# JeffOwOSun/ntm-tracker

Measured on AMD Instinct MI355X. Metric: frames/sec (whole node) VGG16+NTM(128x20) seq_len=20, higher is better.
Workload: dtype f32

## Files before the change

### ntm-tracker_amd/csrc/ntm_phases.h

```cpp
#pragma once
#include "ntm_fwd_args.h"

struct NtmCtl {
    int O, oK, oB, oG, oS, oY, oE, oA, P, PP, ldz, ldh, write_first;
};

__device__ __forceinline__ NtmCtl ntm_ctl(int Md, int R, int Wh, int hid, int SS, int O, int write_first) {
    const int H = R + Wh, K = R * Md + hid;
    NtmCtl d;
    d.O = O;
    d.oK = 0; d.oB = H * Md; d.oG = d.oB + H; d.oS = d.oG + H; d.oY = d.oS + H * SS; d.oE = d.oY + H;
    d.oA = d.oE + Wh * Md; d.P = d.oA + Wh * Md;
    d.PP = (d.P + d.O + 3) & ~3; d.ldz = (K + 1 + 3) & ~3; d.ldh = (hid + 1 + 3) & ~3;
    d.write_first = write_first;
    return d;
}

struct NtmFwdSt {
    int T, N, Md, MP, R, Wh, H, hid, SS, RM;
    int nslB, kperB;
    int nslR, nperR;
    float *sPart, *sM, *sW, *sWg, *sZ, *sU, *sKs, *sPw;
    float* sCn;
    const float* sH;
};

__device__ __forceinline__ NtmFwdSt ntm_fwd_state(float* smem, const NtmLds& L, int T, int N, int Md, int R, int Wh, int hid,
                                                  int SS, int PP, int h_at) {
    NtmFwdSt c;
    c.T = T; c.N = N; c.Md = Md; c.MP = Md | 1; c.R = R; c.Wh = Wh; c.H = R + Wh; c.hid = hid; c.SS = SS; c.RM = R * Md;
    c.nslB = min(max(1, T / (PP >> 2)), hid);
    c.kperB = (hid + c.nslB - 1) / c.nslB;
    c.nslR = min(max(1, T / c.RM), N);
    c.nperR = (N + c.nslR - 1) / c.nslR;
    c.sPart = smem + L.part; c.sM = smem + L.M; c.sW = smem + L.W; c.sWg = smem + L.Wg; c.sZ = smem + L.Z; c.sU = smem + L.U;
    c.sKs = smem + L.Ks; c.sCn = smem + L.Cn; c.sPw = smem + L.Pw;
    c.sH = c.sZ + h_at;
    return c;
}

template <bool SMOOTH>
__device__ __forceinline__ void ntm_fwd_mem_norms(const NtmFwdSt& c, int tid) {
    const int N = c.N, Md = c.Md, MP = c.MP, lane = tid & 63, wave = tid >> 6, nwaves = c.T >> 6;
    const int w0 = (c.hid + 63) >> 6;
    if constexpr (SMOOTH) {
        if (wave >= w0) {
            for (int n = (wave - w0) * 64 + lane; n < N; n += (nwaves - w0) * 64) {
                float s = 0.f;
                for (int m = 0; m < Md; ++m) { const float v = c.sM[n * MP + m]; s += v * v; }
                c.sCn[n] = sqrtf(s);
            }
        }
    } else
    if (wave >= w0) {
        for (int m = wave - w0; m < Md; m += nwaves - w0) {
            float s = 0.f;
            for (int n = lane; n < N; n += 64) { const float v = c.sM[n * MP + m]; s += v * v; }
            s = wave_sum(s);
            if (lane == 0) c.sCn[m] = 1.0f / sqrtf(fmaxf(s, 1e-12f));
        }
    }
}

template <int NB>
__device__ __forceinline__ void ntm_fwd_unpack_partials(const NtmFwdSt& c, const NtmCtl& d, const f32x4* Wa4, int tid) {
    const int ncg = d.PP >> 2;
    if (tid < c.nslB * ncg) {
        const int cg = tid % ncg, ks = tid / ncg;
        const int k0 = ks * c.kperB, k1 = min(c.hid, k0 + c.kperB);
        reinterpret_cast<f32x4*>(c.sPart)[ks * ncg + cg] = ntk_stream_matvec<NB>(Wa4 + cg, ncg, c.sH, k0, k1, c.hid);
    }
}

__device__ __forceinline__ void ntm_fwd_controls(const NtmFwdSt& c, const NtmCtl& d, const NtmFwdArgs& a, int tid, size_t bt) {
    const int hid = c.hid, nslB = c.nslB, PP = d.PP;
    if (tid < PP) {
        float v = a.Wa[(size_t)hid * PP + tid];
        for (int ks = 0; ks < nslB; ++ks) v += c.sPart[ks * PP + tid];
        float r = v;
        if (tid < d.oB) r = ntm_tanh(v);
        else if (tid < d.oG) r = ntm_softplus(v);
        else if (tid < d.oS) r = ntm_sigmoid(v);
        else if (tid < d.oY) r = v;
        else if (tid < d.oE) r = ntm_softplus(v) + 1.0f;
        else if (tid < d.oA) r = ntm_sigmoid(v);
        else if (tid < d.P) r = ntm_tanh(v);
        c.sU[tid] = r;
        if (a.st_u) a.st_u[bt * PP + tid] = r;
        if (tid >= d.P && tid < d.P + d.O) a.logits[bt * d.O + (tid - d.P)] = v;
    }
}

template <bool SMOOTH, int MAXSS>
__device__ __forceinline__ void ntm_fwd_head_wave(const NtmFwdSt& c, const NtmCtl& d, const NtmFwdArgs& a, int h, int lane, size_t bt) {
    const int N = c.N, Md = c.Md, MP = c.MP, H = c.H, SS = c.SS;
    float kss = 0.f;
    for (int m = 0; m < Md; ++m) { const float kv = c.sU[d.oK + h * Md + m]; kss += kv * kv; }
    const float kn = sqrtf(kss);
    if constexpr (SMOOTH) {
        for (int m = lane; m < Md; m += 64) c.sKs[h * Md + m] = c.sU[d.oK + h * Md + m];
    } else {
        const float kinv = 1.0f / sqrtf(fmaxf(kss, 1e-12f));
        if (lane < Md) c.sKs[h * Md + lane] = c.sU[d.oK + h * Md + lane] * kinv * c.sCn[lane];
        for (int m = lane + 64; m < Md; m += 64) c.sKs[h * Md + m] = c.sU[d.oK + h * Md + m] * kinv * c.sCn[m];
    }
    const float beta = c.sU[d.oB + h], g = c.sU[d.oG + h], gamma = c.sU[d.oY + h];
    float swv[MAXSS];
    {
        float mx = -INFINITY;
#pragma unroll
        for (int j = 0; j < MAXSS; ++j) if (j < SS) mx = fmaxf(mx, c.sU[d.oS + h * SS + j]);
        float sum = 0.f;
#pragma unroll
        for (int j = 0; j < MAXSS; ++j) { swv[j] = (j < SS) ? ntm_exp(c.sU[d.oS + h * SS + j] - mx) : 0.f; sum += swv[j]; }
#pragma unroll
        for (int j = 0; j < MAXSS; ++j) swv[j] = swv[j] / sum;
    }
    __builtin_amdgcn_fence(__ATOMIC_ACQ_REL, "wavefront");
    __builtin_amdgcn_wave_barrier();
    float mxv = -INFINITY;
// ... 169 lines not shown
    if (tid < hid) {
        p.G = reinterpret_cast<const f32x4*>(a.st_gates)[bt * hid + tid];
        p.Ct = a.st_c[bt * hid + tid];
        p.Cp = (t > 0) ? a.st_c[(bt - 1) * hid + tid] : c_init[tid];
    }
}

__device__ __forceinline__ void ntm_bwd_commit(const NtmBwdSt& c, const NtmCtl& d, const NtmBwdWho& w, const NtmBwdRecs& p) {
    const int T = c.T, NMd = c.NMd, Md = c.Md, MP = c.MP, hid = c.hid, PP = d.PP, tid = w.tid;
    const bool hn = w.hn, wf = d.write_first != 0;
#pragma unroll
    for (int q = 0; q < MAXM; ++q) {
        const int idx = tid + q * T;
        if (idx < NMd) {
            const int n = idx / Md, m = idx - n * Md;
            c.sMp[n * MP + m] = p.M[q];
            if (wf) c.sMt[n * MP + m] = p.Mt[q];
        }
    }
    if (hn) { c.sWp[tid] = p.Wp; c.sWt[tid] = p.Wt; c.sWc[tid] = p.Wc; c.sWv[tid] = p.Wv; }
    if (tid < PP) { c.sU[tid] = p.U; c.sDU[tid] = p.Dl; }
    if (tid < hid) { reinterpret_cast<f32x4*>(c.sGt)[tid] = p.G; c.sCt[tid] = p.Ct; c.sCp[tid] = p.Cp; }
}

template <class Args>
__device__ __forceinline__ void ntm_bwd_init_carried(const NtmBwdSt& c, const Args& a, int tid) {
    const int b = c.b, T = c.T, NMd = c.NMd, HN = c.HN, Md = c.Md, MP = c.MP, RM = c.R * c.Md;
    for (int i = tid; i < NMd; i += T)
        c.sdM[(i / Md) * MP + (i % Md)] = a.dM_fin ? a.dM_fin[(size_t)b * NMd + i] : 0.f;
    for (int i = tid; i < HN; i += T) c.sdW[i] = a.dw_fin ? a.dw_fin[(size_t)b * HN + i] : 0.f;
    for (int i = tid; i < RM; i += T) c.sdZ[i] = a.dread_fin ? a.dread_fin[(size_t)b * RM + i] : 0.f;
}

template <int NQS>
__device__ __forceinline__ void ntm_red_write(const NtmBwdSt& c, const NtmBwdWho& w, const float (&v)[NQ], int nq, int base) {
#pragma unroll
    for (int q = 0; q < NQ; ++q) {
        if (q < nq) {
            const float s = wave_sum(w.hn ? v[q] : 0.f);
            if (w.hn && w.lane == 0) c.sRed[(w.hh * NQS + base + q) * c.NW + w.wi] = s;
        }
    }
}

template <int NQS>
__device__ __forceinline__ float ntm_red_read(const NtmBwdSt& c, int h, int q) {
    float s = 0.f;
    for (int w = 0; w < c.NW; ++w) s += c.sRed[(h * NQS + q) * c.NW + w];
    return s;
}

template <int MAXT, bool FIX, bool SMOOTH, class Args, class Barrier, class Stamp>
__device__ __forceinline__ void ntm_bwd_heads_step(const NtmBwdSt& c, const NtmCtl& d, const Args& a, const NtmBwdWho& w, size_t bt,
                                                   Barrier&& barrier, Stamp&& stamp) {
    constexpr int NQS = NQT + (SMOOTH ? 1 : 0);
    const int T = c.T, N = c.N, Md = c.Md, MP = c.MP, R = c.R, Wh = c.Wh, H = c.H, SS = c.SS, NMd = c.NMd, PP = d.PP;
    const int nout = c.nout, nslP = c.nslP, nperP = c.nperP, hg4 = c.hg4, nslH = c.nslH, nperH = c.nperH, nslC = c.nslC, nperC = c.nperC;
    const int tid = w.tid, lane = w.lane, hh = w.hh, nn = w.nn;
    const bool hn = w.hn, wf = d.write_first != 0;
    float* const sPart = c.sPart; float* const sdM = c.sdM; float* const sG = c.sG; float* const sMp = c.sMp; float* const sMt = c.sMt;
    float* const sdW = c.sdW; float* const sWp = c.sWp; float* const sWt = c.sWt; float* const sWc = c.sWc; float* const sWv = c.sWv;
    float* const sWg = c.sWg; float* const sDwv = c.sDwv; float* const sDsim = c.sDsim; float* const sU = c.sU; float* const sDU = c.sDU;
    float* const sdZ = c.sdZ; float* const sKhat = c.sKhat; float* const sKs = c.sKs; float* const sKinv = c.sKinv; float* const sKss = c.sKss;
    float* const sCinv = c.sCinv; float* const sCss = c.sCss; float* const sC2 = c.sC2; float* const sDkhat = c.sDkhat;
    float* const sSw = c.sSw; float* const sDmh = c.sDmh;
    const f32x4* const sWaRes4 = c.sWaRes4;
    float* const sRn = sCinv; float* const sRc = sC2;
    f32x4* const sPart4 = reinterpret_cast<f32x4*>(sPart);

    if constexpr (FIX) {
        const int n = tid / 5, m0 = (tid - n * 5) * 4;
        float wt[5];
#pragma unroll
        for (int i = 0; i < 5; ++i) wt[i] = sWt[i * N + n];
        f32x4 dmr = {0.f, 0.f, 0.f, 0.f};
#pragma unroll
        for (int i = 0; i < 4; ++i) dmr += wt[i] * *reinterpret_cast<const f32x4*>(sdZ + i * Md + m0);
#pragma unroll
        for (int e = 0; e < 4; ++e) {
            const int ai = n * MP + m0 + e;
            const float dMt = sdM[ai];
            const float E = 1.0f - wt[4] * sU[d.oE + m0 + e];
            sG[ai] = dMt;
            sdM[ai] = dMt * E + dmr[e];
        }
    } else
    for (int idx = tid; idx < NMd; idx += T) {
        const int n = idx / Md, m = idx - n * Md, ai = n * MP + m;
        float dMt = sdM[ai];
        float dMr = 0.f;
        for (int i = 0; i < R; ++i) dMr += sWt[i * N + n] * sdZ[i * Md + m];
        if (wf) dMt += dMr;
        float E = 1.f;
        for (int j = 0; j < Wh; ++j) E *= (1.0f - sWt[(R + j) * N + n] * sU[d.oE + j * Md + m]);
        sG[ai] = dMt;
        sdM[ai] = dMt * E + (wf ? 0.f : dMr);
    }
    if constexpr (SMOOTH) {
        if (tid < N) {
            float s = 0.f;
            for (int m = 0; m < Md; ++m) { const float v = sMp[tid * MP + m]; s += v * v; }
            sRn[tid] = sqrtf(s);
        }
    } else
    if (tid < nslC * Md) {
        const int m = tid % Md, sl = tid / Md;
        const int n0 = sl * nperC, n1 = min(N, n0 + nperC);
// ... 205 lines not shown
            s = sa + sb;
        }
        sPart[sl * nout + o] = s;
    }
    barrier(5);
    if constexpr (!SMOOTH)
    for (int m = (tid >> 6); m < Md; m += (T >> 6)) {
        float s = 0.f;
        for (int n = lane; n < N; n += 64) s += sDmh[n * MP + m] * sMp[n * MP + m];
        s = wave_sum(s);
        if (lane == 0) {
            const float ci = sCinv[m];
            sC2[m] = (sCss[m] > 1e-12f) ? -ci * ci * ci * s : 0.f;
        }
    }
    if (tid < nout) {
        float s = 0.f;
        for (int sl = 0; sl < (FIX ? 1 : nslP); ++sl) s += sPart[sl * nout + tid];
        if (tid < H * Md) {
            sDkhat[tid] = SMOOTH ? s : s * sCinv[tid % Md];
        } else {
            const int o2 = tid - H * Md;
            const int which = o2 / (Wh * Md);
            const int jm = o2 - which * Wh * Md;
            if (which == 0) { const float e = sU[d.oE + jm]; sDU[d.oE + jm] = s * e * (1.0f - e); }
            else { const float av = sU[d.oA + jm]; sDU[d.oA + jm] = s * (1.0f - av * av); }
        }
    }
    barrier(6);
    if (tid < H * Md) {
        const int h = tid / Md;
        if constexpr (SMOOTH) {
            const float kn = sKinv[h], kv = sU[d.oK + tid];
            const float dk = sDkhat[tid] + ((kn > 0.f) ? kv / kn * ntm_red_read<NQS>(c, h, QR4 + 1) : 0.f);
            sDU[d.oK + tid] = dk * (1.0f - kv * kv);
        } else {
            float dot = 0.f;
            for (int m = 0; m < Md; ++m) dot += sDkhat[h * Md + m] * sU[d.oK + h * Md + m];
            const float ki = sKinv[h];
            const float ck = (sKss[h] > 1e-12f) ? -ki * ki * ki * dot : 0.f;
            const float kv = sU[d.oK + tid];
            const float dk = ki * sDkhat[tid] + kv * ck;
            sDU[d.oK + tid] = dk * (1.0f - kv * kv);
        }
    }
    for (int idx = tid; idx < NMd; idx += T) {
        const int n = idx / Md, m = idx - n * Md, ai = n * MP + m;
        if constexpr (SMOOTH) sdM[ai] += sDmh[ai] + sMp[ai] * sRc[n];
        else sdM[ai] += sCinv[m] * sDmh[ai] + sMp[ai] * sC2[m];
    }
    barrier(7);
    if (tid < PP) a.du[bt * PP + tid] = sDU[tid];

    if (tid < nslH * hg4) {
        const int cg = tid % hg4, sl = tid / hg4;
        const int c0 = sl * nperH, c1 = min(PP, c0 + nperH);
        if constexpr (FIX) {
            f32x4 acc = {0.f, 0.f, 0.f, 0.f};
            const int cs = min(c1, c0 + NTMB_RES_WA);
            const f32x4 str = ntk_stream_matvec_exact<4>(reinterpret_cast<const f32x4*>(a.WaT) + cg, hg4, sDU, cs, c1);
#pragma unroll
            for (int q = 0; q < NTMB_RES_WA; ++q) acc += ((c0 + q < c1) ? sDU[c0 + q] : 0.f) * sWaRes4[q * (nslH * hg4) + tid];
            sPart4[sl * hg4 + cg] = acc + str;
        } else {
            sPart4[sl * hg4 + cg] = ntk_stream_matvec<(MAXT > 768 ? 2 : 4)>(reinterpret_cast<const f32x4*>(a.WaT) + cg, hg4, sDU, c0, c1, PP - 1);
        }
    }
    barrier(8);
}
```

### ntm-tracker_amd/csrc/ntm_seq_bwd.hip

```cpp
#include "ntm_common.h"
#include "ntm_phases.h"
#include <stdlib.h>
#include <type_traits>

#ifdef NTK_CL_PROF
__device__ unsigned long long g_ntm_bwd_prof[16];
#define NTMB_STAMP(i)                                                       \
    do {                                                                    \
        if (blockIdx.x == 0 && tid == 0) {                                  \
            const unsigned long long now_ = __builtin_amdgcn_s_memtime();   \
            s_prof[i] += now_ - s_prof[15];                                 \
            s_prof[15] = now_;                                              \
        }                                                                   \
    } while (0)
extern "C" int ntk_ntm_bwd_prof(unsigned long long* out16) {
    return hipMemcpyFromSymbol(out16, HIP_SYMBOL(g_ntm_bwd_prof), 16 * sizeof(unsigned long long)) == hipSuccess ? NTK_OK : NTK_ERR_HIP;
}
#else
#define NTMB_STAMP(i) do { } while (0)
#endif

struct NtmBwdArgs {
    NtmDims d;
    const float* WrT;
    const float* WaT;
    int ldkT, ldhT;
    const float* M0; const float* w0; const float* cs0;
    const float* st_gates; const float* st_c; const float* st_u;
    const float* st_wc; const float* st_wv; const float* st_w; const float* st_M;
    const float* dlogits;
    const float* dM_fin; const float* dw_fin; const float* dread_fin; const float* dcs_fin;
    float* dgates;
    float* du;
    float* dM0; float* dw0; float* dread0; float* dcs0;
};

static void ntm_bwd_lds(const NtmDims& d, int T, int ldkT, int ldhT, NtmBwdLds& L) {
    const int MP = d.Md | 1, NM = d.N * MP, HN = d.H * d.N;
    const int nout = d.H * d.Md + 2 * d.Wh * d.Md;
    const int nslP = ntm_imin(ntm_imax(1, T / nout), d.N);
    const int nslZ = ntm_imax(1, T / (ldkT / 4));
    const int nslH = ntm_imax(1, T / (ldhT / 4));
    const int nslC = ntm_imax(1, T / d.Md);
    int part = ntm_imax(nslP * nout, nslZ * ldkT);
    part = ntm_imax(part, nslH * ldhT);
    part = ntm_imax(part, nslC * d.Md);
    part = ntm_imax(part, 32 * d.R * d.Md);
    int o = 0;
    auto take = [&](int n) { int r = o; o += ntm_align4(n); return r; };
    L.part = take(part);
    L.dM = take(NM); L.G = take(NM); L.Mp = take(NM); L.Mt = take(d.write_first ? NM : 4);
    L.dW = take(HN); L.Wp = take(HN); L.Wt = take(HN); L.Wc = take(HN); L.Wv = take(HN); L.Wg = take(HN);
    L.Dwv = take(HN); L.Dsim = take(HN);
    L.U = take(d.PP); L.DU = take(d.PP); L.DG = take(4 * d.hid); L.dZ = take(ldkT); L.dC = take(d.hid);
    L.Gt = take(4 * d.hid); L.Ct = take(d.hid); L.Cp = take(d.hid);
    L.Khat = take(d.H * d.Md); L.Ks = take(d.H * d.Md); L.Kinv = take(d.H); L.Kss = take(d.H);
    L.Cinv = take(ntm_norm_floats(d)); L.Css = take(d.Md); L.C2 = take(ntm_norm_floats(d)); L.Dkhat = take(d.H * d.Md);
    L.Sw = take(d.H * d.SS);
    L.Red = take(d.H * (NQT + (d.similarity == NTM_SIM_SMOOTH_COSINE ? 1 : 0)) * (d.N / 64));
    L.Dmh = take(d.N * (d.Md | 1));
    L.total = o;
}

constexpr int BWS_RING = 20, BWS_LAP = 400, BWS_NG = BWS_LAP / 4;
constexpr int kBwdWsGroups[11] = {14, 16, 7, 4, 10, 14, 7, 9, 6, 6, 7};
constexpr int bws_sum(int n) { int s = 0; for (int i = 0; i < n; ++i) s += kBwdWsGroups[i]; return s; }
static_assert(bws_sum(11) == BWS_NG && BWS_LAP % BWS_RING == 0, "one lap per step; the ring's phase is static");

template <int MAXT, bool FIX, bool WS = false, int SIM = NTM_SIM_AS_CODED>
__global__ __launch_bounds__(MAXT) void ntm_seq_bwd_kernel(NtmBwdArgs a, NtmBwdLds L) {
    extern __shared__ __attribute__((aligned(16))) float smem[];
    static_assert(!WS || FIX, "the wave-specialised form exists for the benchmark shape only");
    constexpr bool SMOOTH = SIM == NTM_SIM_SMOOTH_COSINE;
    static_assert(!WS || !SMOOTH, "the wave-specialised form is as coded only");
    const int b = blockIdx.x, tid0 = threadIdx.x, T = FIX ? 640 : blockDim.x;
    const int N = FIX ? 128 : a.d.N, Md = FIX ? 20 : a.d.Md, MP = Md | 1, R = FIX ? 4 : a.d.R, Wh = FIX ? 1 : a.d.Wh;
    const int H = R + Wh, hid = FIX ? 200 : a.d.hid, SS = FIX ? 3 : a.d.SS;
    const int S = a.d.S, RM = R * Md, K = RM + hid, NMd = N * Md, HN = H * N;
    const NtmCtl d = ntm_ctl(Md, R, Wh, hid, SS, FIX ? 2 : a.d.O, FIX ? 0 : a.d.write_first);
    const int PP = d.PP;
    const int ldkT = FIX ? 280 : a.ldkT, ldhT = FIX ? 200 : a.ldhT;
    const NtmBwdSt c = ntm_bwd_state(smem, L, b, S, T, N, Md, R, Wh, hid, SS, PP, ldhT);
    float* const sPart = c.sPart; float* const sdM = c.sdM; float* const sdW = c.sdW; float* const sDG = c.sDG;
    float* const sdZ = c.sdZ; float* const sdC = c.sdC; float* const sGt = c.sGt; float* const sCt = c.sCt; float* const sCp = c.sCp;
    f32x4* sPart4 = reinterpret_cast<f32x4*>(sPart);
    float* sPartH = smem + L.total + 32 + NTMB_RES_WA * 600 * 4;

    if constexpr (WS) {
        if (tid0 >= 640) {
            const int sidx = min(tid0 - 640, 99);
            const int cgs = sidx % 50, sls = sidx / 50;
            const __amdgpu_buffer_rsrc_t wrs = __builtin_amdgcn_make_buffer_rsrc(const_cast<float*>(a.WrT + 80), 0,
                                                                                  (800 * 280 - 80) * (int)sizeof(float), 0x00020000);
            const unsigned voff = (unsigned)cgs * 16u + (unsigned)sls * (unsigned)(BWS_LAP * 280 * sizeof(float));
            auto wrow = [&](int r) { return __builtin_bit_cast(f32x4, __builtin_amdgcn_raw_buffer_load_b128(wrs, voff, r * (280 * (int)sizeof(float)), 0)); };
            const float* dgp = sDG + BWS_LAP * sls;
            constexpr int G0 = kBwdWsGroups[9] + kBwdWsGroups[10];
            f32x4 ring[BWS_RING];
#pragma unroll
            for (int q = 0; q < BWS_RING; ++q) ring[(4 * G0 + q) % BWS_RING] = wrow((4 * G0 + q) % BWS_LAP);
            f32x4 acc = {0.f, 0.f, 0.f, 0.f};
            if (sls == 0 && a.dcs_fin) acc = *reinterpret_cast<const f32x4*>(a.dcs_fin + (size_t)b * 2 * hid + hid + 4 * cgs);
            auto group = [&](auto gc) {
                constexpr int r = 4 * decltype(gc)::value;
                const f32x4 hv = *reinterpret_cast<const f32x4*>(dgp + r);
#pragma unroll
                for (int q = 0; q < 4; ++q) {
                    acc += hv[q] * ring[(r + q) % BWS_RING];
                    ring[(r + q) % BWS_RING] = wrow((r + q + BWS_RING) % BWS_LAP);
                }
                __builtin_amdgcn_sched_barrier(0);
            };
            auto finish_lap = [&]() {
                constexpr int c0 = G0, c1 = c0 + kBwdWsGroups[0], c2 = c1 + kBwdWsGroups[1], c3 = c2 + kBwdWsGroups[2],
                              c4 = c3 + kBwdWsGroups[3], c5 = c4 + kBwdWsGroups[4], c6 = c5 + kBwdWsGroups[5],
                              c7 = c6 + kBwdWsGroups[6], c8 = c7 + kBwdWsGroups[7];
                static_assert(c8 + kBwdWsGroups[8] == BWS_NG, "lap");
                ntk_static_for<c0, c1>(group); __syncthreads();
                ntk_static_for<c1, c2>(group); __syncthreads();
                ntk_static_for<c2, c3>(group); __syncthreads();
                ntk_static_for<c3, c4>(group); __syncthreads();
                ntk_static_for<c4, c5>(group); __syncthreads();
                ntk_static_for<c5, c6>(group); __syncthreads();
                ntk_static_for<c6, c7>(group); __syncthreads();
                ntk_static_for<c7, c8>(group); __syncthreads();
                ntk_static_for<c8, BWS_NG>(group);
                reinterpret_cast<f32x4*>(sPartH)[sls * 50 + cgs] = acc;
                acc = f32x4{0.f, 0.f, 0.f, 0.f};
            };
            __syncthreads();
            __syncthreads();
            for (int t = S - 1; t >= 0; --t) {
                finish_lap();
                __syncthreads();
                __syncthreads();
                ntk_static_for<0, kBwdWsGroups[9]>(group);
                __syncthreads();
                ntk_static_for<kBwdWsGroups[9], G0>(group);
                __syncthreads();
            }
            finish_lap();
            __syncthreads();
            return;
        }
    }

    const int kg4 = ldkT >> 2, hg4 = c.hg4;
    const int nslZ = max(1, T / kg4), nperZ = (4 * hid + nslZ - 1) / nslZ;
    const int nslH = c.nslH, nperH = c.nperH;

    ntm_bwd_init_carried(c, a, tid0);
    for (int i = RM + tid0; i < ldkT; i += T) sdZ[i] = (i < K && a.dcs_fin) ? a.dcs_fin[(size_t)b * 2 * hid + hid + (i - RM)] : 0.f;
    for (int i = tid0; i < hid; i += T) sdC[i] = a.dcs_fin ? a.dcs_fin[(size_t)b * 2 * hid + i] : 0.f;
    if constexpr (WS) {
        for (int i = tid0; i < 4 * hid; i += T) sDG[i] = 0.f;
    }
    NtmBwdRecs rec = {};
    const float* const c_init = a.cs0 + (size_t)b * 2 * hid;
    {
        const NtmBwdWho w = ntm_bwd_who(tid0, N, H);
        ntm_bwd_prefetch(c, d, a, w, rec, S - 1, c_init);
        ntm_bwd_commit(c, d, w, rec);
    }
    __syncthreads();

    if constexpr (FIX) {
        if (tid0 < nslH * hg4) {
            const int cg = tid0 % hg4, sl = tid0 / hg4;
            const int c0 = sl * nperH, c1 = min(PP, c0 + nperH);
            f32x4* wl = reinterpret_cast<f32x4*>(smem + L.total + 32);
            for (int q = 0; q < NTMB_RES_WA; ++q)
                wl[q * (nslH * hg4) + tid0] = (c0 + q < c1) ? reinterpret_cast<const f32x4*>(a.WaT)[(size_t)(c0 + q) * hg4 + cg] : f32x4{0.f, 0.f, 0.f, 0.f};
        }
        __syncthreads();
    }
    constexpr int NTMB_RES_B11 = 5;
    f32x4 wres11[NTMB_RES_B11];
    if constexpr (WS) {
        const int cg = tid0 % 20, sl = tid0 / 20;
#pragma unroll
        for (int q = 0; q < NTMB_RES_B11; ++q) wres11[q] = reinterpret_cast<const f32x4*>(a.WrT)[(size_t)(sl * 25 + q) * kg4 + cg];
    }
#ifdef NTK_CL_PROF
    unsigned long long* s_prof = reinterpret_cast<unsigned long long*>(smem + L.total);
    if (threadIdx.x == 0) { for (int i = 0; i < 15; ++i) s_prof[i] = 0; s_prof[15] = __builtin_amdgcn_s_memtime(); }
#endif
    for (int t = S - 1; t >= 0; --t) {
        int tid_op = tid0;
        asm volatile("" : "+v"(tid_op));
        const NtmBwdWho w = ntm_bwd_who(tid_op, N, H);
        const int tid = w.tid;
        const size_t bt = (size_t)b * S + t;
        if (t > 0) ntm_bwd_prefetch(c, d, a, w, rec, t - 1, c_init);

        ntm_bwd_heads_step<MAXT, FIX, SMOOTH>(c, d, a, w, bt, [&](int i) { __syncthreads(); NTMB_STAMP(i); }, [&](int i) { NTMB_STAMP(i); });
        if (tid < hid) {
            float dh = WS ? sPartH[tid] + sPartH[hid + tid] : sdZ[RM + tid];
            for (int sl = 0; sl < nslH; ++sl) dh += sPart[sl * ldhT + tid];
            const f32x4 g = reinterpret_cast<const f32x4*>(sGt)[tid];
            const float gi = g[0], gj = g[1], gf = g[2], go = g[3];
            const float tc = tanhf(sCt[tid]);
            const float dct = sdC[tid] + dh * go * (1.0f - tc * tc);
            f32x4 dg;
            dg[0] = dct * gj * gi * (1.0f - gi);
            dg[1] = dct * gi * (1.0f - gj * gj);
            dg[2] = dct * sCp[tid] * gf * (1.0f - gf);
            dg[3] = dh * tc * go * (1.0f - go);
            sdC[tid] = dct * gf;
            reinterpret_cast<f32x4*>(sDG)[tid] = dg;
            reinterpret_cast<f32x4*>(a.dgates)[bt * hid + tid] = dg;
        }
        __syncthreads();
        NTMB_STAMP(9);
        if constexpr (WS) {
            const int cg = tid % 20, sl = tid / 20;
            f32x4 acc = {0.f, 0.f, 0.f, 0.f};
#pragma unroll
            for (int q = 0; q < NTMB_RES_B11; ++q) acc += sDG[sl * 25 + q] * wres11[q];
            sPart4[sl * 20 + cg] = ntk_stream_matvec_exact<4>(reinterpret_cast<const f32x4*>(a.WrT) + cg, kg4, sDG, sl * 25 + NTMB_RES_B11, sl * 25 + 25, acc);
        } else if (tid < nslZ * kg4) {
            const int cg = tid % kg4, sl = tid / kg4;
            const int r0 = sl * nperZ, r1 = min(4 * hid, r0 + nperZ);
            sPart4[sl * kg4 + cg] = ntk_stream_matvec<(MAXT > 768 ? 2 : 8)>(reinterpret_cast<const f32x4*>(a.WrT) + cg, kg4, sDG, r0, r1, 4 * hid - 1);
        }
        __syncthreads();
        NTMB_STAMP(10);
        if constexpr (WS) {
            if (tid < RM) {
                float s = 0.f;
#pragma unroll 8
                for (int sl = 0; sl < 32; ++sl) s += sPart[sl * RM + tid];
                sdZ[tid] = s;
            }
        } else if (tid < K) {
            float s = 0.f;
            for (int sl = 0; sl < nslZ; ++sl) s += sPart[sl * ldkT + tid];
            sdZ[tid] = s;
        }
        if (t > 0) ntm_bwd_commit(c, d, w, rec);
        __syncthreads();
        NTMB_STAMP(11);
    }

#ifdef NTK_CL_PROF
    if (blockIdx.x == 0 && threadIdx.x == 0) for (int i = 0; i < 16; ++i) g_ntm_bwd_prof[i] = s_prof[i];
#endif
    for (int i = tid0; i < NMd; i += T) a.dM0[(size_t)b * NMd + i] = sdM[(i / Md) * MP + (i % Md)];
    for (int i = tid0; i < HN; i += T) a.dw0[(size_t)b * HN + i] = sdW[i];
// ... 80 lines not shown
                                    int similarity,
                                    int ldkT, int ldhT, int* fwd_kernel, int* fwd_threads, int* bwd_kernel, int* bwd_threads) {
    NTM_REQUIRE_SIMILARITY(similarity, "ntk_ntm_seq_plan");
    NtmDims d;
    ntm_fill_dims(d, B, 1, N, Md, R, Wh, hid, shift_range, O, write_first, similarity);
    if (ldkT <= 0) ldkT = ntm_align4(d.K);
    if (ldhT <= 0) ldhT = ntm_align4(hid);
    NtmBwdPlan pb;
    NtmFwdPlan pf;
    const bool bwd = ntm_bwd_plan(d, ldkT, ldhT, pb, "ntk_ntm_seq_bwd") == NTK_OK;
    const bool fwd = ntm_fwd_plan(d, pf, "ntk_ntm_seq_fwd") == NTK_OK;
    if (fwd_kernel) *fwd_kernel = fwd ? pf.kernel : 0;
    if (fwd_threads) *fwd_threads = fwd ? pf.T : 0;
    if (bwd_kernel) *bwd_kernel = bwd ? pb.kernel : 0;
    if (bwd_threads) *bwd_threads = bwd ? pb.threads : 0;
    return (fwd ? NTK_NTM_PLAN_FWD : 0) | (bwd ? NTK_NTM_PLAN_BWD : 0);
}

extern "C" int ntk_ntm_seq_plan(int B, int N, int Md, int R, int Wh, int hid, int shift_range, int O, int write_first,
                                int ldkT, int ldhT, int* fwd_kernel, int* fwd_threads, int* bwd_kernel, int* bwd_threads) {
    return ntk_ntm_seq_plan_sim(B, N, Md, R, Wh, hid, shift_range, O, write_first, NTM_SIM_AS_CODED, ldkT, ldhT, fwd_kernel, fwd_threads,
                                bwd_kernel, bwd_threads);
}

extern "C" int ntk_ntm_seq_bwd_sim(int B, int S, int N, int Md, int R, int Wh, int hid, int shift_range, int O,
                               int write_first, int similarity,
                               const float* WrT, int ldkT, const float* WaT, int ldhT,
                               const float* M0, const float* w0, const float* cs0,
                               const float* st_gates, const float* st_c, const float* st_u,
                               const float* st_wc, const float* st_wv, const float* st_w, const float* st_M,
                               const float* dlogits,
                               const float* dM_fin, const float* dw_fin, const float* dread_fin, const float* dcs_fin,
                               float* dgates, float* du, float* dM0, float* dw0, float* dread0, float* dcs0,
                               void* stream) {
    NTM_REQUIRE_SIMILARITY(similarity, "ntk_ntm_seq_bwd");
    NtmBwdArgs a;
    ntm_fill_dims(a.d, B, S, N, Md, R, Wh, hid, shift_range, O, write_first, similarity);
    NtmBwdPlan p;
    int rc = ntm_bwd_plan(a.d, ldkT, ldhT, p, "ntk_ntm_seq_bwd");
    if (rc != NTK_OK) return rc;
    NTK_REQUIRE(WrT && WaT && M0 && w0 && cs0 && st_gates && st_c && st_u && st_wc && st_wv && st_w && st_M &&
                    dlogits && dgates && du && dM0 && dw0 && dread0 && dcs0,
                NTK_ERR_BAD_PTR, "ntk_ntm_seq_bwd: null pointer");
    NTK_REQUIRE(ntk_aligned16(WrT) && ntk_aligned16(WaT) && ntk_aligned16(st_gates) && ntk_aligned16(dgates),
                NTK_ERR_BAD_PTR, "ntk_ntm_seq_bwd: WrT/WaT/st_gates/dgates must be 16-byte aligned");
    a.WrT = WrT; a.WaT = WaT; a.ldkT = ldkT; a.ldhT = ldhT; a.M0 = M0; a.w0 = w0; a.cs0 = cs0;
    a.st_gates = st_gates; a.st_c = st_c; a.st_u = st_u; a.st_wc = st_wc; a.st_wv = st_wv; a.st_w = st_w; a.st_M = st_M;
    a.dlogits = dlogits; a.dM_fin = dM_fin; a.dw_fin = dw_fin; a.dread_fin = dread_fin; a.dcs_fin = dcs_fin;
    a.dgates = dgates; a.du = du; a.dM0 = dM0; a.dw0 = dw0; a.dread0 = dread0; a.dcs0 = dcs0;
    {
        static NtkLdsAttrCache lds_cache;
        const void* const ks[] = {(const void*)ntm_seq_bwd_kernel<768, false>, (const void*)ntm_seq_bwd_kernel<1024, false>, (const void*)ntm_seq_bwd_kernel<768, true>,
                                  (const void*)ntm_seq_bwd_kernel<768, true, true>,
                                  (const void*)ntm_seq_bwd_kernel<768, false, false, NTM_SIM_SMOOTH_COSINE>,
                                  (const void*)ntm_seq_bwd_kernel<1024, false, false, NTM_SIM_SMOOTH_COSINE>,
                                  (const void*)ntm_seq_bwd_kernel<768, true, false, NTM_SIM_SMOOTH_COSINE>};
        const int rc_lds = ntk_raise_lds_limit(lds_cache, ks, 7, "ntk_ntm_seq_bwd");
        if (rc_lds != NTK_OK) return rc_lds;
    }
    const hipStream_t st = (hipStream_t)stream;
    if (similarity == NTM_SIM_SMOOTH_COSINE) {
        constexpr int SC = NTM_SIM_SMOOTH_COSINE;
        if (p.kernel == NTK_NTM_BWD_FIX) ntm_seq_bwd_kernel<768, true, false, SC><<<B, p.threads, p.lds_bytes, st>>>(a, p.L);
        else if (p.kernel == NTK_NTM_BWD_GENERIC768) ntm_seq_bwd_kernel<768, false, false, SC><<<B, p.threads, p.lds_bytes, st>>>(a, p.L);
        else if (p.kernel == NTK_NTM_BWD_GENERIC1024) ntm_seq_bwd_kernel<1024, false, false, SC><<<B, p.threads, p.lds_bytes, st>>>(a, p.L);
        else NTK_REQUIRE(false, NTK_ERR_UNSUPPORTED, "ntk_ntm_seq_bwd: kernel %d has no smooth-cosine form", p.kernel);
    } else
    if (p.kernel == NTK_NTM_BWD_WS) ntm_seq_bwd_kernel<768, true, true><<<B, p.threads, p.lds_bytes, st>>>(a, p.L);
    else if (p.kernel == NTK_NTM_BWD_FIX) ntm_seq_bwd_kernel<768, true><<<B, p.threads, p.lds_bytes, st>>>(a, p.L);
    else if (p.kernel == NTK_NTM_BWD_GENERIC768) ntm_seq_bwd_kernel<768, false><<<B, p.threads, p.lds_bytes, st>>>(a, p.L);
    else ntm_seq_bwd_kernel<1024, false><<<B, p.threads, p.lds_bytes, st>>>(a, p.L);
    NTK_CHECK_LAUNCH("ntk_ntm_seq_bwd");
    return NTK_OK;
}

extern "C" int ntk_ntm_seq_bwd(int B, int S, int N, int Md, int R, int Wh, int hid, int shift_range, int O,
                               int write_first,
                               const float* WrT, int ldkT, const float* WaT, int ldhT,
                               const float* M0, const float* w0, const float* cs0,
                               const float* st_gates, const float* st_c, const float* st_u,
                               const float* st_wc, const float* st_wv, const float* st_w, const float* st_M,
                               const float* dlogits,
                               const float* dM_fin, const float* dw_fin, const float* dread_fin, const float* dcs_fin,
                               float* dgates, float* du, float* dM0, float* dw0, float* dread0, float* dcs0,
                               void* stream) {
    return ntk_ntm_seq_bwd_sim(B, S, N, Md, R, Wh, hid, shift_range, O, write_first, NTM_SIM_AS_CODED, WrT, ldkT, WaT, ldhT, M0, w0, cs0,
                               st_gates, st_c, st_u, st_wc, st_wv, st_w, st_M, dlogits, dM_fin, dw_fin, dread_fin, dcs_fin,
                               dgates, du, dM0, dw0, dread0, dcs0, stream);
}
```

### ntm-tracker_amd/csrc/ntm_seq_fwd_ws.hip

```cpp
#include "ntm_phases.h"
#include <stdlib.h>
#include <type_traits>

#ifdef NTK_CL_PROF
__device__ unsigned long long g_ntm_ws_prof[2][16];
#define WS_STAMP(role, i)                                                   \
    do {                                                                    \
        if (prof_on) {                                                      \
            const unsigned long long now_ = __builtin_amdgcn_s_memtime();   \
            s_prof[(role) * 16 + (i)] += now_ - s_prof[(role) * 16 + 15];   \
            s_prof[(role) * 16 + 15] = now_;                                \
        }                                                                   \
    } while (0)
extern "C" int ntk_ntm_ws_prof(unsigned long long* out32) {
    return hipMemcpyFromSymbol(out32, HIP_SYMBOL(g_ntm_ws_prof), 32 * sizeof(unsigned long long)) == hipSuccess ? NTK_OK : NTK_ERR_HIP;
}
#else
#define WS_STAMP(role, i) do { } while (0)
#endif
#define WS_BARRIER(role, i) do { WS_STAMP(role, 2 * (i)); __syncthreads(); WS_STAMP(role, 2 * (i) + 1); } while (0)

namespace {

constexpr int WN = 128, WMd = 20, WMP = 21, WR = 4, WH = 5, Whid = 200, WSS = 3, WRM = 80, WK = 280, WO = 2;
constexpr int TC = 512, TA = 768;
constexpr int RESQ = 20, RESL = 20;
constexpr int NG = Whid / 4;

template <int RING, int P3, int P4, int P5, int P6, int P7>
__global__ __launch_bounds__(TA) void ntm_seq_fwd_ws_kernel(NtmFwdArgs a, NtmLds L) {
    extern __shared__ __attribute__((aligned(16))) float smem[];
    constexpr int PFIN = P3 + P4 + P5 + P6 + P7;
    static_assert(PFIN >= 0 && PFIN <= NG && Whid % RING == 0, "groups per lap; the ring's phase is static when it divides the lap");
    const int b = blockIdx.x, tid0 = threadIdx.x;
    const int S = a.d.S;
    constexpr int N = WN, Md = WMd, MP = WMP, R = WR, Wh = 1, H = WH, hid = Whid, SS = WSS, RM = WRM, K = WK;

    float* sPart = smem + L.part;
    float* sM = smem + L.M;
    float* sW = smem + L.W;
    float* sZ = smem + L.Z;
    float* sC = smem + L.C;
    f32x4* sWres4 = reinterpret_cast<f32x4*>(smem + L.total + 32);
    f32x4* sPartH4 = reinterpret_cast<f32x4*>(smem + L.total + 32 + RESL * 400 * 4);
    f32x4* sPart4 = reinterpret_cast<f32x4*>(sPart);
    const f32x4* Wr4 = reinterpret_cast<const f32x4*>(a.Wr);
    const f32x4* Wa4 = reinterpret_cast<const f32x4*>(a.Wa);

    for (int i = tid0; i < N * Md; i += TA) sM[(i / Md) * MP + (i % Md)] = a.M0[(size_t)b * N * Md + i];
    for (int i = tid0; i < H * N; i += TA) sW[i] = a.w0[(size_t)b * H * N + i];
    for (int i = tid0; i < RM; i += TA) sZ[i] = a.read0[(size_t)b * RM + i];
    for (int i = tid0; i < hid; i += TA) {
        sC[i] = a.cs0[(size_t)b * 2 * hid + i];
        sZ[RM + i] = a.cs0[(size_t)b * 2 * hid + hid + i];
    }
#ifdef NTK_CL_PROF
    unsigned long long* s_prof = reinterpret_cast<unsigned long long*>(smem + L.total + 32 + RESL * 400 * 4 + 4 * hid);
    const bool prof_on = blockIdx.x == 0 && (tid0 == 0 || tid0 == TC);
    if (prof_on) { const int ro = tid0 == 0 ? 0 : 16; for (int i = 0; i < 15; ++i) s_prof[ro + i] = 0; }
#endif
    __syncthreads();
#ifdef NTK_CL_PROF
    if (prof_on) s_prof[(tid0 == 0 ? 0 : 16) + 15] = __builtin_amdgcn_s_memtime();
#endif

    if (tid0 >= TC) {
        const int j = min(tid0 - TC, hid - 1);
        const __amdgpu_buffer_rsrc_t wrs = __builtin_amdgcn_make_buffer_rsrc(const_cast<float*>(a.Wr + (size_t)RM * 4 * hid), 0,
                                                                              hid * 4 * hid * (int)sizeof(float), 0x00020000);
        const unsigned voff = (unsigned)j * 16u;
        auto wrow = [&](int r) { return __builtin_bit_cast(f32x4, __builtin_amdgcn_raw_buffer_load_b128(wrs, voff, r * (4 * hid * (int)sizeof(float)), 0)); };
        const float* sHp = sZ + RM;
        f32x4 ring[RING];
        f32x4 acc = {0.f, 0.f, 0.f, 0.f};
#pragma unroll 1
        for (int r0 = 0; r0 < 4 * PFIN; r0 += 4) {
            f32x4 w[4];
#pragma unroll
            for (int q = 0; q < 4; ++q) w[q] = wrow(r0 + q);
            const f32x4 hv = *reinterpret_cast<const f32x4*>(sHp + r0);
#pragma unroll
            for (int q = 0; q < 4; ++q) acc += hv[q] * w[q];
        }
#pragma unroll
        for (int q = 0; q < RING; ++q) ring[(4 * PFIN + q) % RING] = wrow((4 * PFIN + q) % hid);
        auto group = [&](auto gc) {
            constexpr int r = 4 * decltype(gc)::value;
            const f32x4 hv = *reinterpret_cast<const f32x4*>(sHp + r);
#pragma unroll
            for (int q = 0; q < 4; ++q) {
                acc += hv[q] * ring[(r + q) % RING];
                ring[(r + q) % RING] = wrow((r + q + RING) % hid);
            }
            __builtin_amdgcn_sched_barrier(0);
        };
        for (int t = 0; t < S; ++t) {
            ntk_static_for<PFIN, NG>(group);
            sPartH4[j] = acc;
            acc = f32x4{0.f, 0.f, 0.f, 0.f};
            WS_BARRIER(1, 0);
            WS_BARRIER(1, 1);
            ntk_static_for<0, P3>(group);
            WS_BARRIER(1, 2);
            ntk_static_for<P3, P3 + P4>(group);
            WS_BARRIER(1, 3);
            ntk_static_for<P3 + P4, P3 + P4 + P5>(group);
            WS_BARRIER(1, 4);
            ntk_static_for<P3 + P4 + P5, P3 + P4 + P5 + P6>(group);
            WS_BARRIER(1, 5);
            ntk_static_for<P3 + P4 + P5 + P6, PFIN>(group);
            WS_BARRIER(1, 6);
        }
#ifdef NTK_CL_PROF
        if (prof_on) for (int i = 0; i < 16; ++i) g_ntm_ws_prof[1][i] = s_prof[16 + i];
#endif
        return;
    }

    constexpr int T = TC;
    const NtmCtl d = ntm_ctl(Md, R, Wh, hid, SS, WO, 0);
    const NtmFwdSt c = ntm_fwd_state(smem, L, T, N, Md, R, Wh, hid, SS, d.PP, RM);
    f32x4 wres[RESQ];
    if (tid0 < 2 * hid) {
        const int j = tid0 % hid, k0 = (tid0 / hid) * (RESQ + RESL);
#pragma unroll
        for (int q = 0; q < RESQ; ++q) wres[q] = Wr4[(size_t)(k0 + q) * hid + j];
        for (int q = 0; q < RESL; ++q) sWres4[q * (2 * hid) + tid0] = Wr4[(size_t)(k0 + RESQ + q) * hid + j];
    }
    for (int t = 0; t < S; ++t) {
        int tid_op = tid0;
        asm volatile("" : "+v"(tid_op));
        const int tid = tid_op;
        const int lane = tid & 63, wave = tid >> 6;
        const size_t bt = (size_t)b * S + t;
        f32x4 xg = {0.f, 0.f, 0.f, 0.f};
        if (tid < hid) {
            xg = reinterpret_cast<const f32x4*>(a.xproj)[bt * hid + tid];
            xg += Wr4[(size_t)K * hid + tid];
        }
        if (a.st_z) {
            for (int i = tid; i < d.ldz; i += T) a.st_z[bt * d.ldz + i] = (i < K) ? sZ[i] : (i == K ? 1.f : 0.f);
        }
        if (tid < 2 * hid) {
            const int k0 = (tid / hid) * (RESQ + RESL);
            f32x4 acc = {0.f, 0.f, 0.f, 0.f};
#pragma unroll
            for (int q = 0; q < RESQ; ++q) acc += sZ[k0 + q] * wres[q];
#pragma unroll 4
            for (int q = 0; q < RESL; ++q) acc += sZ[k0 + RESQ + q] * sWres4[q * (2 * hid) + tid];
            sPart4[tid] = acc;
        }
        WS_BARRIER(0, 0);
        if (tid < hid) {
            const f32x4 g = ((xg + sPart4[tid]) + sPart4[hid + tid]) + sPartH4[tid];
            const float gi = ntm_sigmoid(g[0]);
            const float gj = ntm_tanh(g[1]);
            const float gf = ntm_sigmoid(g[2]);
            const float go = ntm_sigmoid(g[3]);
            const float c2 = sC[tid] * gf + gi * gj;
            const float h2 = ntm_tanh(c2) * go;
            sC[tid] = c2;
            sZ[RM + tid] = h2;
            if (a.st_gates) {
                f32x4 ga = {gi, gj, gf, go};
                reinterpret_cast<f32x4*>(a.st_gates)[bt * hid + tid] = ga;
                a.st_c[bt * hid + tid] = c2;
            }
            if (a.st_h) a.st_h[bt * d.ldh + tid] = h2;
        } else if (a.st_h && tid < d.ldh) {
            a.st_h[bt * d.ldh + tid] = (tid == hid) ? 1.f : 0.f;
        }
        ntm_fwd_mem_norms<false>(c, tid);
        WS_BARRIER(0, 1);
        ntm_fwd_unpack_partials<4>(c, d, Wa4, tid);
        WS_BARRIER(0, 2);
        ntm_fwd_controls(c, d, a, tid, bt);
        WS_BARRIER(0, 3);
        if (wave < H) ntm_fwd_head_wave<false, SS>(c, d, a, wave, lane, bt);
        else if (wave == H && lane == 0 && a.outputs) ntm_fwd_output_softmax(c, d, a, bt);
        WS_BARRIER(0, 4);
        ntm_fwd_read_partials(c, tid);
        WS_BARRIER(0, 5);
        for (int idx = tid; idx < N * Md; idx += T) {
            const int n = idx / Md, m = idx - n * Md;
            const float ww = sW[R * N + n];
            const float nm = sM[n * MP + m] * (1.0f - ww * c.sU[d.oE + m]) + ww * c.sU[d.oA + m];
            sM[n * MP + m] = nm;
            if (a.st_M) a.st_M[bt * N * Md + idx] = nm;
        }
        ntm_fwd_read_finish(c, a, tid, bt);
        WS_BARRIER(0, 6);
    }

#ifdef NTK_CL_PROF
    if (prof_on) for (int i = 0; i < 16; ++i) g_ntm_ws_prof[0][i] = s_prof[i];
#endif
    for (int i = tid0; i < N * Md; i += T) a.M_out[(size_t)b * N * Md + i] = sM[(i / Md) * MP + (i % Md)];
    for (int i = tid0; i < H * N; i += T) a.w_out[(size_t)b * H * N + i] = sW[i];
    for (int i = tid0; i < RM; i += T) a.read_out[(size_t)b * RM + i] = sZ[i];
    for (int i = tid0; i < hid; i += T) {
        a.cs_out[(size_t)b * 2 * hid + i] = sC[i];
        a.cs_out[(size_t)b * 2 * hid + hid + i] = sZ[RM + i];
    }
}

}

bool ntm_seq_fwd_ws_takes(const NtmDims& d) {
    return d.N == WN && d.Md == WMd && d.R == WR && d.Wh == 1 && d.hid == Whid && d.SS == WSS && d.O == WO && !d.write_first;
}

int ntm_seq_fwd_ws_plan(const NtmDims& d, NtmLds& L, size_t& lds_bytes) {
    ntm_fwd_lds(d, TC, L);
    lds_bytes = (size_t)L.total * sizeof(float) + 128 + (size_t)RESL * 400 * sizeof(f32x4) + (size_t)Whid * sizeof(f32x4);
#ifdef NTK_CL_PROF
    lds_bytes += 256;
#endif
    return TA;
}

int ntm_seq_fwd_ws_launch(const NtmFwdArgs& a, const NtmLds& L, size_t lds_bytes, void* stream) {
    const char* split_env = getenv("NTK_NTM_WS_SPLIT");
    const int split = split_env ? atoi(split_env) : 0;
    typedef void (*kern_t)(NtmFwdArgs, NtmLds);
    static const kern_t ks[] = {ntm_seq_fwd_ws_kernel<20, 5, 5, 23, 7, 7>, ntm_seq_fwd_ws_kernel<20, 5, 5, 21, 6, 7>,
                                ntm_seq_fwd_ws_kernel<20, 4, 5, 20, 6, 6>, ntm_seq_fwd_ws_kernel<25, 5, 5, 23, 7, 7>,
                                ntm_seq_fwd_ws_kernel<25, 5, 5, 21, 6, 7>, ntm_seq_fwd_ws_kernel<25, 4, 5, 20, 6, 6>,
                                ntm_seq_fwd_ws_kernel<10, 5, 5, 23, 7, 7>, ntm_seq_fwd_ws_kernel<20, 6, 6, 24, 7, 7>,
                                ntm_seq_fwd_ws_kernel<25, 6, 6, 24, 7, 7>, ntm_seq_fwd_ws_kernel<20, 3, 4, 18, 5, 5>};
    constexpr int NK = (int)(sizeof(ks) / sizeof(ks[0]));
    static NtkLdsAttrCache lds_cache;
    const int rc = ntk_raise_lds_limit(lds_cache, reinterpret_cast<const void* const*>(ks), NK, "ntk_ntm_seq_fwd");
    if (rc != NTK_OK) return rc;
    ks[(split >= 0 && split < NK) ? split : 0]<<<a.d.B, TA, lds_bytes, (hipStream_t)stream>>>(a, L);
    NTK_CHECK_LAUNCH("ntk_ntm_seq_fwd(ws)");
    return NTK_OK;
}
```

Measured before the change: 13230.

## Hold slices of Wa/WaT in helper-wave registers for the fwd and bwd matvecs

In the wave-specialised forward and backward NTM kernels, the otherwise idle helper waves (threads beyond the compute group) now keep whole slices of the Wa / WaT weight matrices in registers. Each step they compute those partial matvec items themselves, and the compute threads skip the matching items, which removes part of the per-step weight streaming from global memory. The forward path also changes its default ring size and phase split, and the backward loop is reshaped so the last lap runs inside the loop. The cost is more register pressure in the helper waves, which could force spills or slow their own streaming work. Env vars keep the old variants selectable.

```diff
diff --git a/ntm-tracker_amd/csrc/ntm_phases.h b/ntm-tracker_amd/csrc/ntm_phases.h
--- a/ntm-tracker_amd/csrc/ntm_phases.h
+++ b/ntm-tracker_amd/csrc/ntm_phases.h
@@ -63,9 +63,9 @@
 }
 
 template <int NB>
-__device__ __forceinline__ void ntm_fwd_unpack_partials(const NtmFwdSt& c, const NtmCtl& d, const f32x4* Wa4, int tid) {
+__device__ __forceinline__ void ntm_fwd_unpack_partials(const NtmFwdSt& c, const NtmCtl& d, const f32x4* Wa4, int tid, int first = 0) {
     const int ncg = d.PP >> 2;
-    if (tid < c.nslB * ncg) {
+    if (tid >= first && tid < c.nslB * ncg) {
         const int cg = tid % ncg, ks = tid / ncg;
         const int k0 = ks * c.kperB, k1 = min(c.hid, k0 + c.kperB);
         reinterpret_cast<f32x4*>(c.sPart)[ks * ncg + cg] = ntk_stream_matvec<NB>(Wa4 + cg, ncg, c.sH, k0, k1, c.hid);
@@ -341,7 +341,7 @@
 
 template <int MAXT, bool FIX, bool SMOOTH, class Args, class Barrier, class Stamp>
 __device__ __forceinline__ void ntm_bwd_heads_step(const NtmBwdSt& c, const NtmCtl& d, const Args& a, const NtmBwdWho& w, size_t bt,
-                                                   Barrier&& barrier, Stamp&& stamp) {
+                                                   Barrier&& barrier, Stamp&& stamp, int b9_first = 0) {
     constexpr int NQS = NQT + (SMOOTH ? 1 : 0);
     const int T = c.T, N = c.N, Md = c.Md, MP = c.MP, R = c.R, Wh = c.Wh, H = c.H, SS = c.SS, NMd = c.NMd, PP = d.PP;
     const int nout = c.nout, nslP = c.nslP, nperP = c.nperP, hg4 = c.hg4, nslH = c.nslH, nperH = c.nperH, nslC = c.nslC, nperC = c.nperC;
@@ -653,7 +653,7 @@
     barrier(7);
     if (tid < PP) a.du[bt * PP + tid] = sDU[tid];
 
-    if (tid < nslH * hg4) {
+    if (tid >= b9_first && tid < nslH * hg4) {
         const int cg = tid % hg4, sl = tid / hg4;
         const int c0 = sl * nperH, c1 = min(PP, c0 + nperH);
         if constexpr (FIX) {
diff --git a/ntm-tracker_amd/csrc/ntm_seq_bwd.hip b/ntm-tracker_amd/csrc/ntm_seq_bwd.hip
--- a/ntm-tracker_amd/csrc/ntm_seq_bwd.hip
+++ b/ntm-tracker_amd/csrc/ntm_seq_bwd.hip
@@ -66,11 +66,13 @@
 constexpr int kBwdWsGroups[11] = {14, 16, 7, 4, 10, 14, 7, 9, 6, 6, 7};
 constexpr int bws_sum(int n) { int s = 0; for (int i = 0; i < n; ++i) s += kBwdWsGroups[i]; return s; }
 static_assert(bws_sum(11) == BWS_NG && BWS_LAP % BWS_RING == 0, "one lap per step; the ring's phase is static");
-
-template <int MAXT, bool FIX, bool WS = false, int SIM = NTM_SIM_AS_CODED>
+constexpr int BWS_B9_ITEMS = 12 * 50, BWS_B9_ROWS = 15, BWS_B9_STREAMED = BWS_B9_ROWS - NTMB_RES_WA;
+
+template <int MAXT, bool FIX, bool WS = false, int SIM = NTM_SIM_AS_CODED, int RES9 = 0>
 __global__ __launch_bounds__(MAXT) void ntm_seq_bwd_kernel(NtmBwdArgs a, NtmBwdLds L) {
     extern __shared__ __attribute__((aligned(16))) float smem[];
     static_assert(!WS || FIX, "the wave-specialised form exists for the benchmark shape only");
+    static_assert(RES9 == 0 || (WS && 128 * RES9 <= 11 * 50), "resident items of B9: stream waves only, full 15-row slices only");
     constexpr bool SMOOTH = SIM == NTM_SIM_SMOOTH_COSINE;
     static_assert(!WS || !SMOOTH, "the wave-specialised form is as coded only");
     const int b = blockIdx.x, tid0 = threadIdx.x, T = FIX ? 640 : blockDim.x;
@@ -108,6 +110,32 @@
                 for (int q = 0; q < 4; ++q) {
                     acc += hv[q] * ring[(r + q) % BWS_RING];
                     ring[(r + q) % BWS_RING] = wrow((r + q + BWS_RING) % BWS_LAP);
+                }
+                __builtin_amdgcn_sched_barrier(0);
+            };
+            constexpr int NW9 = RES9 > 0 ? RES9 : 1;
+            f32x4 w9[NW9][BWS_B9_STREAMED];
+            const int item0 = tid0 - 640;
+            if constexpr (RES9 > 0) {
+#pragma unroll
+                for (int k = 0; k < RES9; ++k) {
+                    const int i = item0 + 128 * k;
+#pragma unroll
+                    for (int q = 0; q < BWS_B9_STREAMED; ++q)
+                        w9[k][q] = reinterpret_cast<const f32x4*>(a.WaT)[(size_t)((i / 50) * BWS_B9_ROWS + NTMB_RES_WA + q) * 50 + i % 50];
+                }
+            }
+            auto b9_items = [&]() {
+#pragma unroll
+                for (int k = 0; k < RES9; ++k) {
+                    const int i = item0 + 128 * k;
+                    const float* du = c.sDU + (i / 50) * BWS_B9_ROWS;
+                    f32x4 res = {0.f, 0.f, 0.f, 0.f}, str = {0.f, 0.f, 0.f, 0.f};
+#pragma unroll
+                    for (int q = 0; q < BWS_B9_STREAMED; ++q) str += du[NTMB_RES_WA + q] * w9[k][q];
+#pragma unroll
+                    for (int q = 0; q < NTMB_RES_WA; ++q) res += du[q] * c.sWaRes4[q * BWS_B9_ITEMS + i];
+                    sPart4[i] = res + str;
                 }
                 __builtin_amdgcn_sched_barrier(0);
             };
@@ -124,23 +152,23 @@
                 ntk_static_for<c5, c6>(group); __syncthreads();
                 ntk_static_for<c6, c7>(group); __syncthreads();
                 ntk_static_for<c7, c8>(group); __syncthreads();
+                if constexpr (RES9 > 0) b9_items();
                 ntk_static_for<c8, BWS_NG>(group);
                 reinterpret_cast<f32x4*>(sPartH)[sls * 50 + cgs] = acc;
                 acc = f32x4{0.f, 0.f, 0.f, 0.f};
             };
             __syncthreads();
             __syncthreads();
-            for (int t = S - 1; t >= 0; --t) {
+            for (int t = S; ; --t) {
                 finish_lap();
                 __syncthreads();
+                if (t == 0) break;
                 __syncthreads();
                 ntk_static_for<0, kBwdWsGroups[9]>(group);
                 __syncthreads();
                 ntk_static_for<kBwdWsGroups[9], G0>(group);
                 __syncthreads();
             }
-            finish_lap();
-            __syncthreads();
             return;
         }
     }
@@ -193,7 +221,7 @@
         const size_t bt = (size_t)b * S + t;
         if (t > 0) ntm_bwd_prefetch(c, d, a, w, rec, t - 1, c_init);
 
-        ntm_bwd_heads_step<MAXT, FIX, SMOOTH>(c, d, a, w, bt, [&](int i) { __syncthreads(); NTMB_STAMP(i); }, [&](int i) { NTMB_STAMP(i); });
+        ntm_bwd_heads_step<MAXT, FIX, SMOOTH>(c, d, a, w, bt, [&](int i) { __syncthreads(); NTMB_STAMP(i); }, [&](int i) { NTMB_STAMP(i); }, 128 * RES9);
         if (tid < hid) {
             float dh = WS ? sPartH[tid] + sPartH[hid + tid] : sdZ[RM + tid];
             for (int sl = 0; sl < nslH; ++sl) dh += sPart[sl * ldhT + tid];
@@ -380,10 +408,11 @@
         static NtkLdsAttrCache lds_cache;
         const void* const ks[] = {(const void*)ntm_seq_bwd_kernel<768, false>, (const void*)ntm_seq_bwd_kernel<1024, false>, (const void*)ntm_seq_bwd_kernel<768, true>,
                                   (const void*)ntm_seq_bwd_kernel<768, true, true>,
+                                  (const void*)ntm_seq_bwd_kernel<768, true, true, NTM_SIM_AS_CODED, 1>,
                                   (const void*)ntm_seq_bwd_kernel<768, false, false, NTM_SIM_SMOOTH_COSINE>,
                                   (const void*)ntm_seq_bwd_kernel<1024, false, false, NTM_SIM_SMOOTH_COSINE>,
                                   (const void*)ntm_seq_bwd_kernel<768, true, false, NTM_SIM_SMOOTH_COSINE>};
-        const int rc_lds = ntk_raise_lds_limit(lds_cache, ks, 7, "ntk_ntm_seq_bwd");
+        const int rc_lds = ntk_raise_lds_limit(lds_cache, ks, (int)(sizeof(ks) / sizeof(ks[0])), "ntk_ntm_seq_bwd");
         if (rc_lds != NTK_OK) return rc_lds;
     }
     const hipStream_t st = (hipStream_t)stream;
@@ -394,7 +423,11 @@
         else if (p.kernel == NTK_NTM_BWD_GENERIC1024) ntm_seq_bwd_kernel<1024, false, false, SC><<<B, p.threads, p.lds_bytes, st>>>(a, p.L);
         else NTK_REQUIRE(false, NTK_ERR_UNSUPPORTED, "ntk_ntm_seq_bwd: kernel %d has no smooth-cosine form", p.kernel);
     } else
-    if (p.kernel == NTK_NTM_BWD_WS) ntm_seq_bwd_kernel<768, true, true><<<B, p.threads, p.lds_bytes, st>>>(a, p.L);
+    if (p.kernel == NTK_NTM_BWD_WS) {
+        const char* res_env = getenv("NTK_NTM_WS_RESIDENT");
+        if (res_env && res_env[0] == '0') ntm_seq_bwd_kernel<768, true, true><<<B, p.threads, p.lds_bytes, st>>>(a, p.L);
+        else ntm_seq_bwd_kernel<768, true, true, NTM_SIM_AS_CODED, 1><<<B, p.threads, p.lds_bytes, st>>>(a, p.L);
+    }
     else if (p.kernel == NTK_NTM_BWD_FIX) ntm_seq_bwd_kernel<768, true><<<B, p.threads, p.lds_bytes, st>>>(a, p.L);
     else if (p.kernel == NTK_NTM_BWD_GENERIC768) ntm_seq_bwd_kernel<768, false><<<B, p.threads, p.lds_bytes, st>>>(a, p.L);
     else ntm_seq_bwd_kernel<1024, false><<<B, p.threads, p.lds_bytes, st>>>(a, p.L);
diff --git a/ntm-tracker_amd/csrc/ntm_seq_fwd_ws.hip b/ntm-tracker_amd/csrc/ntm_seq_fwd_ws.hip
--- a/ntm-tracker_amd/csrc/ntm_seq_fwd_ws.hip
+++ b/ntm-tracker_amd/csrc/ntm_seq_fwd_ws.hip
@@ -26,8 +26,11 @@
 constexpr int TC = 512, TA = 768;
 constexpr int RESQ = 20, RESL = 20;
 constexpr int NG = Whid / 4;
-
-template <int RING, int P3, int P4, int P5, int P6, int P7>
+constexpr int WPP = (WH * WMd + 3 * WH + WH * WSS + 2 * WMd + WO + 3) & ~3, WNCG = WPP / 4, WNSLB = TC / WNCG;
+constexpr int WKPER = (Whid + WNSLB - 1) / WNSLB, WS_RES_ITEMS = TA - TC;
+static_assert(WPP == 172 && WNSLB == 11 && WKPER == 19 && WS_RES_ITEMS <= (Whid / WKPER) * WNCG, "the resident items are whole 19-row slices");
+
+template <int RING, bool RES, int P3, int P4, int P5, int P6, int P7>
 __global__ __launch_bounds__(TA) void ntm_seq_fwd_ws_kernel(NtmFwdArgs a, NtmLds L) {
     extern __shared__ __attribute__((aligned(16))) float smem[];
     constexpr int PFIN = P3 + P4 + P5 + P6 + P7;
@@ -73,6 +76,13 @@
         const float* sHp = sZ + RM;
         f32x4 ring[RING];
         f32x4 acc = {0.f, 0.f, 0.f, 0.f};
+        constexpr int NWA = RES ? WKPER : 1;
+        f32x4 wa[NWA];
+        const int item = tid0 - TC, ha = (item / WNCG) * WKPER;
+        if constexpr (RES) {
+#pragma unroll
+            for (int q = 0; q < WKPER; ++q) wa[q] = Wa4[(size_t)(ha + q) * WNCG + item % WNCG];
+        }
 #pragma unroll 1
         for (int r0 = 0; r0 < 4 * PFIN; r0 += 4) {
             f32x4 w[4];
@@ -100,6 +110,13 @@
             acc = f32x4{0.f, 0.f, 0.f, 0.f};
             WS_BARRIER(1, 0);
             WS_BARRIER(1, 1);
+            if constexpr (RES) {
+                f32x4 pa = {0.f, 0.f, 0.f, 0.f};
+#pragma unroll
+                for (int q = 0; q < WKPER; ++q) pa += sHp[ha + q] * wa[q];
+                sPart4[item] = pa;
+                __builtin_amdgcn_sched_barrier(0);
+            }
             ntk_static_for<0, P3>(group);
             WS_BARRIER(1, 2);
             ntk_static_for<P3, P3 + P4>(group);
@@ -172,7 +189,7 @@
         }
         ntm_fwd_mem_norms<false>(c, tid);
         WS_BARRIER(0, 1);
-        ntm_fwd_unpack_partials<4>(c, d, Wa4, tid);
+        ntm_fwd_unpack_partials<4>(c, d, Wa4, tid, RES ? WS_RES_ITEMS : 0);
         WS_BARRIER(0, 2);
         ntm_fwd_controls(c, d, a, tid, bt);
         WS_BARRIER(0, 3);
@@ -220,19 +237,20 @@
 }
 
 int ntm_seq_fwd_ws_launch(const NtmFwdArgs& a, const NtmLds& L, size_t lds_bytes, void* stream) {
+    const char* res_env = getenv("NTK_NTM_WS_RESIDENT");
     const char* split_env = getenv("NTK_NTM_WS_SPLIT");
+    const bool res = !(res_env && res_env[0] == '0');
     const int split = split_env ? atoi(split_env) : 0;
     typedef void (*kern_t)(NtmFwdArgs, NtmLds);
-    static const kern_t ks[] = {ntm_seq_fwd_ws_kernel<20, 5, 5, 23, 7, 7>, ntm_seq_fwd_ws_kernel<20, 5, 5, 21, 6, 7>,
-                                ntm_seq_fwd_ws_kernel<20, 4, 5, 20, 6, 6>, ntm_seq_fwd_ws_kernel<25, 5, 5, 23, 7, 7>,
-                                ntm_seq_fwd_ws_kernel<25, 5, 5, 21, 6, 7>, ntm_seq_fwd_ws_kernel<25, 4, 5, 20, 6, 6>,
-                                ntm_seq_fwd_ws_kernel<10, 5, 5, 23, 7, 7>, ntm_seq_fwd_ws_kernel<20, 6, 6, 24, 7, 7>,
-                                ntm_seq_fwd_ws_kernel<25, 6, 6, 24, 7, 7>, ntm_seq_fwd_ws_kernel<20, 3, 4, 18, 5, 5>};
-    constexpr int NK = (int)(sizeof(ks) / sizeof(ks[0]));
+    constexpr int NRES = 4, NOLD = 2;
+    static const kern_t ks[NRES + NOLD] = {ntm_seq_fwd_ws_kernel<10, true, 2, 5, 23, 7, 7>, ntm_seq_fwd_ws_kernel<10, true, 1, 5, 23, 7, 7>,
+                                           ntm_seq_fwd_ws_kernel<10, true, 0, 5, 23, 7, 7>, ntm_seq_fwd_ws_kernel<10, true, 5, 5, 23, 7, 7>,
+                                           ntm_seq_fwd_ws_kernel<20, false, 5, 5, 23, 7, 7>, ntm_seq_fwd_ws_kernel<10, false, 5, 5, 23, 7, 7>};
     static NtkLdsAttrCache lds_cache;
-    const int rc = ntk_raise_lds_limit(lds_cache, reinterpret_cast<const void* const*>(ks), NK, "ntk_ntm_seq_fwd");
+    const int rc = ntk_raise_lds_limit(lds_cache, reinterpret_cast<const void* const*>(ks), NRES + NOLD, "ntk_ntm_seq_fwd");
     if (rc != NTK_OK) return rc;
-    ks[(split >= 0 && split < NK) ? split : 0]<<<a.d.B, TA, lds_bytes, (hipStream_t)stream>>>(a, L);
+    const int which = res ? ((split >= 0 && split < NRES) ? split : 0) : NRES + ((split >= 0 && split < NOLD) ? split : 0);
+    ks[which]<<<a.d.B, TA, lds_bytes, (hipStream_t)stream>>>(a, L);
     NTK_CHECK_LAUNCH("ntk_ntm_seq_fwd(ws)");
     return NTK_OK;
 }
```

New measurement: 13290 (median of 6 runs). No clear change (+0.4%).
